# richa-batra/ParticleRobotSimulations

Hardware: AMD Instinct MI355X
Metric: particle-steps/sec at 10^6 bots; achieved HBM GB/s vs peak; 1/2/4/8-GPU ensemble (higher is better)
Workload: dtype f32

## Files before the change

### include/particlebot_hip.h

```cpp
#ifndef PARTICLEBOT_HIP_H
#define PARTICLEBOT_HIP_H

#include <stddef.h>

#include "particlebot_kernel.h"

#ifdef __cplusplus
extern "C" {
#endif

struct pbGraphicsResource;

enum { PB_RNG_COUNTER = 0, PB_RNG_XORWOW_CURAND = 1, PB_RNG_XORWOW_ROCRAND = 2 };

typedef struct pbRngState {
  unsigned d;
  unsigned v[5];
  int boxmuller_flag;
  int kind;
  float boxmuller_extra;
  float reserved[3];
} pbRngState;

int pbSetRngKind(int kind);
// ... 36 lines not shown
void updateCol(float *rad, float *col, int nCells, float *pos, float *phase, int *dead);
void collide(float *newVel, float *absForce_a, float *absForce_r, float *sortedPos, float *sortedVel,
             float *sortedRad, uint *gridParticlebotIndex, uint *cellStart, uint *cellEnd, uint nCells,
             uint numCells, float deltaTime);
void calcCOG(float *pos, float *temppos, float *temppos1, int nCells, float time, int hist_steps,
             float hist_int);
void sortParticlebots(uint *dGridParticlebotHash, uint *dGridParticlebotIndex, uint nCells);


typedef struct pbSim pbSim;

enum {
  PB_OK = 0,
  PB_ERR_HIP = 1,
  PB_ERR_ARG = 2,
  PB_ERR_NO_DEVICE = 3
};

typedef struct pbSimStats {
  unsigned long long steps;
  unsigned long long fused_launches;
  unsigned long long plain_launches;
  unsigned long long state_launches;
  unsigned long long resorts;
  unsigned long long phase_updates;
  unsigned long long resident_launches;
} pbSimStats;

const char *pbGetLastErrorString(void);

int pbGetDevice(int *device);
int pbSetDevice(int device);
int pbDevicePciBusId(int device, char *out, int cap);

int pbSimCreate(pbSim **out, const SimParams *params, float wallHalf);
void pbSimDestroy(pbSim *sim);

int pbSimCreateBatch(pbSim **out, const SimParams *params, int nsims, float wallHalf);
int pbSimBatchSize(pbSim *sim, unsigned *nsims, unsigned *nbots);
int pbSimSetStateOf(pbSim *sim, unsigned member, const float *pos, const float *vel, const float *rad,
                    const float *phase, const int *dead);
int pbSimSetStateRangeOf(pbSim *sim, unsigned member, unsigned start, unsigned count, const float *pos,
                         const float *vel, const float *rad, const float *phase, const int *dead);
int pbSimGetStateOf(pbSim *sim, unsigned member, float *pos, float *vel, float *rad, float *phase, int *dead,
                    float *absForce_a, float *absForce_r);
int pbSimGetLayoutOf(pbSim *sim, unsigned member, unsigned *orig, unsigned *keys, int *sorted);
int pbSimSetLayoutOf(pbSim *sim, unsigned member, const unsigned *orig, const unsigned *keys);
int pbSimSetForcesOf(pbSim *sim, unsigned member, const float *absForce_a, const float *absForce_r);
int pbSimCentroids(pbSim *sim, double *cxcy);
int pbSimCentroidSums(pbSim *sim, float *sumxy);
int pbSimGetColorsOf(pbSim *sim, unsigned member, float *rgba);
int pbSimSetCentroidTrail(pbSim *sim, int on);
int pbSimGetCentroidTrailOf(pbSim *sim, unsigned member, float *xy, float *times, unsigned *records);

int pbSimSetState(pbSim *sim, const float *pos, const float *vel, const float *rad, const float *phase,
                  const int *dead);
int pbSimGetState(pbSim *sim, float *pos, float *vel, float *rad, float *phase, int *dead,
                  float *absForce_a, float *absForce_r);
int pbSimSetTime(pbSim *sim, float time);
int pbSimGetTime(pbSim *sim, float *time);
int pbSimGetPhaseDraws(pbSim *sim, unsigned *draws);
int pbSimSetPhaseDraws(pbSim *sim, unsigned draws);

int pbSimStep(pbSim *sim, float deltaTime, float sort_interval, int nsteps, int *steps_done);
int pbSimStepTimed(pbSim *sim, float deltaTime, float sort_interval, int nsteps, int *steps_done,
                   float *elapsed_ms);
int pbSimStepTimedWall(pbSim *sim, float deltaTime, float sort_interval, int nsteps, int *steps_done,
                       float *elapsed_ms, double *wall_ms);
int pbSimSynchronize(pbSim *sim);

int pbSimCentroid(pbSim *sim, double *cx, double *cy);
int pbSimGetStats(pbSim *sim, pbSimStats *stats);
int pbSimSetResortEveryStep(pbSim *sim, int on);

int pbSimSetMinDistanceMode(pbSim *sim, int mode);
int pbSetMinDistanceMode(int mode);
int pbGetMinDistanceMode(void);

float pbHostSqrtThreshold(float c);

int pbSimSetForceVariant(pbSim *sim, int variant);
int pbSimSetForceSums(pbSim *sim, int mode);
int pbSimSetLanesPerBot(pbSim *sim, int lanes);
int pbSimSetResident(pbSim *sim, int mode);

int pbSimSetRng(pbSim *sim, int kind);
int pbSimGetRngStatesOf(pbSim *sim, unsigned member, pbRngState *states);

typedef struct pbForceForm {
  int flat;
  int lanes_per_bot;
  int attraction_sums;
  int offsets64;
} pbForceForm;
int pbForceFormCount(void);
int pbForceFormGet(int index, pbForceForm *form);
int pbSimSelectForceForm(pbSim *sim, int index);
int pbSimForceKernelName(pbSim *sim, char *buf, size_t cap);
int pbForceFormKernelName(int index, int payload, char *buf, size_t cap);

int pbSimSetStreamWalk(pbSim *sim, int mode);
int pbSimGetStreamWalkTrips(pbSim *sim, unsigned long long *row_by_row, unsigned long long *flattened);

typedef struct pbSimConfig {
  int force_variant;
  int force_kind;
  int lanes_per_bot;
  int resident;
  int fast_math_ok;
  int payload;
  int rng;
  int offsets64;
  int attraction_sums;
  int dead_sum_form;
  int stream_walk;
} pbSimConfig;
int pbSimGetConfig(pbSim *sim, pbSimConfig *cfg);

typedef struct pbClockSample pbClockSample;
int pbClockSampleBegin(pbClockSample **out, double seconds);
int pbClockSampleEnd(pbClockSample *sample, double *mhz, double *seconds_sampled);

int pbSelfTest(unsigned long long div_samples, unsigned long long *sqrt_checked,
               unsigned long long *sqrt_mismatches, unsigned long long *div_checked,
               unsigned long long *div_mismatches);

int pbSelfTestHoldThreshold(float c, unsigned long long *checked, unsigned long long *mismatches);
int pbSelfTestPairGeometry(unsigned first_slice, unsigned slices, unsigned long long *checked,
                           unsigned long long *mismatches);
int pbSelfTestDivision(unsigned first_slice, unsigned slices, unsigned long long *checked,
                       unsigned long long *mismatches);

#ifdef __cplusplus
}
#endif
#endif
```

### particlerobotsimulations_amd/__init__.py

```python
import ctypes as C

import numpy as np

from . import _capi
from ._capi import SimParams, make_params, pbSimConfig, pbSimStats

__all__ = ["Sim", "Ensemble", "DeviceArray", "legacy", "SimParams", "make_params", "library_paths", "self_test"]


def self_test(div_samples=1 << 32):
    vals = [C.c_ulonglong() for _ in range(4)]
    _capi.check(_capi.lib().pbSelfTest(int(div_samples), *[C.byref(v) for v in vals]), "pbSelfTest")
    keys = ("sqrt_checked", "sqrt_mismatches", "div_checked", "div_mismatches")
    return {k: int(v.value) for k, v in zip(keys, vals)}


def self_test_hold_threshold(c):
    checked, bad = C.c_ulonglong(), C.c_ulonglong()
    _capi.check(_capi.lib().pbSelfTestHoldThreshold(float(c), C.byref(checked), C.byref(bad)), "pbSelfTestHoldThreshold")
    return {"checked": checked.value, "mismatches": bad.value}


def self_test_pair_geometry(first_slice=0, slices=64):
    checked, bad = C.c_ulonglong(), C.c_ulonglong()
# ... 197 lines not shown
        return out

    @property
    def time(self):
        t = C.c_float()
        _capi.check(_capi.lib().pbSimGetTime(self._h, C.byref(t)))
        return t.value

    @time.setter
    def time(self, t):
        _capi.check(_capi.lib().pbSimSetTime(self._h, float(t)))

    @property
    def phase_draws(self):
        d = C.c_uint()
        _capi.check(_capi.lib().pbSimGetPhaseDraws(self._h, C.byref(d)))
        return d.value

    @phase_draws.setter
    def phase_draws(self, d):
        _capi.check(_capi.lib().pbSimSetPhaseDraws(self._h, int(d)))

    def step(self, nsteps, dt=0.01, sort_interval=180.0):
        done = C.c_int()
        _capi.check(_capi.lib().pbSimStep(self._h, dt, sort_interval, int(nsteps), C.byref(done)), "pbSimStep")
        return done.value

    def step_timed(self, nsteps, dt=0.01, sort_interval=180.0):
        done = C.c_int()
        ms = C.c_float()
        _capi.check(_capi.lib().pbSimStepTimed(self._h, dt, sort_interval, int(nsteps), C.byref(done),
                                               C.byref(ms)), "pbSimStepTimed")
        return done.value, ms.value

    def step_timed_wall(self, nsteps, dt=0.01, sort_interval=180.0):
        done, ms, wall = C.c_int(), C.c_float(), C.c_double()
        _capi.check(_capi.lib().pbSimStepTimedWall(self._h, dt, sort_interval, int(nsteps), C.byref(done), C.byref(ms),
                                                   C.byref(wall)), "pbSimStepTimedWall")
        return done.value, ms.value, wall.value

    def synchronize(self):
        _capi.check(_capi.lib().pbSimSynchronize(self._h))

    def centroid(self):
        cx, cy = C.c_double(), C.c_double()
        _capi.check(_capi.lib().pbSimCentroid(self._h, C.byref(cx), C.byref(cy)), "pbSimCentroid")
        return cx.value, cy.value

    def stats(self):
        s = pbSimStats()
        _capi.check(_capi.lib().pbSimGetStats(self._h, C.byref(s)))
        return {k: int(getattr(s, k)) for k, _ in pbSimStats._fields_}

    def config(self):
        c = pbSimConfig()
        _capi.check(_capi.lib().pbSimGetConfig(self._h, C.byref(c)))
        return {k: int(getattr(c, k)) for k, _ in pbSimConfig._fields_}

    def force_kernel_name(self):
        buf = C.create_string_buffer(2048)
        _capi.check(_capi.lib().pbSimForceKernelName(self._h, buf, len(buf)), "pbSimForceKernelName")
        return buf.value.decode()

    def set_force_variant(self, variant):
        _capi.check(_capi.lib().pbSimSetForceVariant(self._h, int(variant)))

    def set_stream_walk(self, mode):
        _capi.check(_capi.lib().pbSimSetStreamWalk(self._h, int(mode)), "pbSimSetStreamWalk")

    def stream_walk_trips(self):
        a, b = C.c_ulonglong(0), C.c_ulonglong(0)
        _capi.check(_capi.lib().pbSimGetStreamWalkTrips(self._h, C.byref(a), C.byref(b)), "pbSimGetStreamWalkTrips")
        return a.value, b.value

    def set_force_sums(self, mode):
        _capi.check(_capi.lib().pbSimSetForceSums(self._h, int(mode)))

    def select_force_form(self, index):
        _capi.check(_capi.lib().pbSimSelectForceForm(self._h, int(index)), "pbSimSelectForceForm")

    def set_lanes_per_bot(self, lanes):
        _capi.check(_capi.lib().pbSimSetLanesPerBot(self._h, int(lanes)))

    def set_resident(self, mode):
        _capi.check(_capi.lib().pbSimSetResident(self._h, int(mode)))

    def set_resort_every_step(self, on):
        _capi.check(_capi.lib().pbSimSetResortEveryStep(self._h, 1 if on else 0))

    def colors(self, member=0):
        out = np.empty((self.n, 4), np.float32)
        _capi.check(_capi.lib().pbSimGetColorsOf(self._h, int(member), _capi.np_ptr(out)), "pbSimGetColorsOf")
        return out

    def set_centroid_trail(self, on):
        _capi.check(_capi.lib().pbSimSetCentroidTrail(self._h, 1 if on else 0), "pbSimSetCentroidTrail")

    def centroid_trail(self, member=0):
        steps = int(self.params.centroid_steps)
        xy = np.empty((steps, 2), np.float32)
        times = np.empty(steps, np.float32)
        rec = C.c_uint(0)
        _capi.check(_capi.lib().pbSimGetCentroidTrailOf(self._h, int(member), _capi.np_ptr(xy), _capi.np_ptr(times),
                                                        C.byref(rec)), "pbSimGetCentroidTrailOf")
        return xy, times, int(rec.value)


class Ensemble(Sim):

    def __init__(self, params_list, wall_half=0.0, keepalive=None):
        self._keep = keepalive
        self.nsims = len(params_list)
        arr = (SimParams * self.nsims)(*params_list)
        self.params = params_list[0]
        self.n = int(params_list[0].nCells)
        h = C.c_void_p()
        _capi.check(_capi.lib().pbSimCreateBatch(C.byref(h), arr, self.nsims, float(wall_half)), "pbSimCreateBatch")
        self._h = h

    def set_state_of(self, member, pos=None, vel=None, rad=None, phase=None, dead=None):
        n = self.n
        pos = self._in(pos, np.float32, 2 * n)
        vel = self._in(vel, np.float32, 2 * n)
        rad = self._in(rad, np.float32, n)
        phase = self._in(phase, np.float32, n)
        dead = self._in(dead, np.int32, n)
        _capi.check(_capi.lib().pbSimSetStateOf(self._h, int(member), _capi.np_ptr(pos), _capi.np_ptr(vel),
                                                _capi.np_ptr(rad), _capi.np_ptr(phase), _capi.np_ptr(dead)),
                    "pbSimSetStateOf")

    def get_state_of(self, member):
        n = self.n
        out = {
            "pos": np.empty((n, 2), np.float32), "vel": np.empty((n, 2), np.float32),
            "rad": np.empty(n, np.float32), "phase": np.empty(n, np.float32),
            "dead": np.empty(n, np.int32), "absForce_a": np.empty(n, np.float32),
            "absForce_r": np.empty(n, np.float32),
        }
        _capi.check(_capi.lib().pbSimGetStateOf(self._h, int(member), *[_capi.np_ptr(out[k]) for k in
                                                                        ("pos", "vel", "rad", "phase", "dead",
                                                                         "absForce_a", "absForce_r")]),
                    "pbSimGetStateOf")
        if not self.config()["attraction_sums"]:
            out["absForce_a"] = None
        return out

    def centroids(self):
        out = np.empty((self.nsims, 2), np.float64)
        _capi.check(_capi.lib().pbSimCentroids(self._h, out.ctypes.data_as(C.POINTER(C.c_double))), "pbSimCentroids")
        return out

    def centroid_sums(self):
        out = np.empty((self.nsims, 2), np.float32)
        _capi.check(_capi.lib().pbSimCentroidSums(self._h, out.ctypes.data_as(C.POINTER(C.c_float))), "pbSimCentroidSums")
        return out
```

### particlerobotsimulations_amd/_capi.py

```python
import ctypes as C
import os

import numpy as np

_PKG = os.path.dirname(os.path.abspath(__file__))
LIB_DIR = os.path.join(_PKG, "lib")
HIP_SO = os.path.join(LIB_DIR, "libparticlebot_hip.so")
HOST_SO = os.path.join(LIB_DIR, "libparticlebot_host.so")

PB_MAX_OBSTACLES = 10
PB_OK = 0


class uint2(C.Structure):
    _fields_ = [("x", C.c_uint), ("y", C.c_uint)]


class float2(C.Structure):
    _fields_ = [("x", C.c_float), ("y", C.c_float)]


class SimParams(C.Structure):
    _fields_ = [
        ("gridSize", uint2), ("numCells", C.c_uint),
        ("_pad0", C.c_uint),
        ("worldOrigin", float2), ("cellSize", float2),
        ("nCells", C.c_uint), ("nDead", C.c_int), ("maxParticlebotsPerCell", C.c_uint),
        ("gravity", C.c_float), ("spring", C.c_float), ("damping", C.c_float), ("shear", C.c_float),
        ("attraction", C.c_float), ("boundaryDamping", C.c_float), ("friction", C.c_float),
        ("massFactor", C.c_float), ("frictionFactor", C.c_float), ("radFactor", C.c_float),
        ("attractionFactor", C.c_float),
        ("constraint", C.c_float), ("constraint_contraction", C.c_float),
        ("centroid_steps", C.c_int), ("centroid_int", C.c_float), ("centroid_radius", C.c_float),
        ("light_x", C.c_float), ("light_y", C.c_float), ("phase_update_interval", C.c_float),
        ("control", C.c_int), ("config", C.c_int),
        ("min_radius", C.c_float), ("max_radius", C.c_float), ("rise_period", C.c_float),
        ("freq", C.c_float),
        ("nobstacles", C.c_int),
        ("x1obs", C.POINTER(C.c_float)), ("x2obs", C.POINTER(C.c_float)),
        ("y1obs", C.POINTER(C.c_float)), ("y2obs", C.POINTER(C.c_float)),
        ("n_cir_obstacles", C.c_int),
        ("x_cir_obs", C.POINTER(C.c_float)), ("y_cir_obs", C.POINTER(C.c_float)),
        ("r_cir_obs", C.POINTER(C.c_float)),
        ("Nx", C.c_int), ("phase_std", C.c_float), ("seed", C.c_uint),
        ("light_shadow", C.c_uint), ("testing", C.c_uint), ("constrained_contraction", C.c_uint),
        ("display_shadow", C.c_uint), ("time_to_dead", C.c_float), ("max_time", C.c_float),
    ]


class pbRngState(C.Structure):
    _fields_ = [("d", C.c_uint), ("v", C.c_uint * 5), ("boxmuller_flag", C.c_int), ("kind", C.c_int),
                ("boxmuller_extra", C.c_float), ("reserved", C.c_float * 3)]


PB_RNG_COUNTER, PB_RNG_XORWOW_CURAND, PB_RNG_XORWOW_ROCRAND = 0, 1, 2


class pbSimStats(C.Structure):
    _fields_ = [("steps", C.c_ulonglong), ("fused_launches", C.c_ulonglong),
                ("plain_launches", C.c_ulonglong), ("state_launches", C.c_ulonglong),
                ("resorts", C.c_ulonglong), ("phase_updates", C.c_ulonglong),
                ("resident_launches", C.c_ulonglong)]


class pbSimConfig(C.Structure):
    _fields_ = [("force_variant", C.c_int), ("force_kind", C.c_int), ("lanes_per_bot", C.c_int),
                ("resident", C.c_int), ("fast_math_ok", C.c_int), ("payload", C.c_int), ("rng", C.c_int), ("offsets64", C.c_int),
                ("attraction_sums", C.c_int), ("dead_sum_form", C.c_int), ("stream_walk", C.c_int)]


class pbForceForm(C.Structure):
    _fields_ = [("flat", C.c_int), ("lanes_per_bot", C.c_int), ("attraction_sums", C.c_int), ("offsets64", C.c_int)]


_VP = C.c_void_p
_F = C.c_float
_U = C.c_uint
_I = C.c_int
SYMBOLS = {
    "cudaInit": (None, [_I, _VP]),
    "cudaGLInit": (None, [_I, _VP]),
    "allocateArray": (None, [C.POINTER(_VP), C.c_size_t]),
    "freeArray": (None, [_VP]),
    "threadSync": (None, []),
    "copyArrayFromDevice": (None, [_VP, _VP, _VP, _I]),
    "copyArrayToDevice": (None, [_VP, _VP, _I, _I]),
    "registerGLBufferObject": (None, [_U, C.POINTER(_VP)]),
    "unregisterGLBufferObject": (None, [_VP]),
    "mapGLBufferObject": (_VP, [C.POINTER(_VP)]),
    "unmapGLBufferObject": (None, [_VP]),
    "pbCreateBuffer": (_U, [C.c_size_t]),
    "pbBufferSubData": (None, [_U, C.c_size_t, C.c_size_t, _VP]),
    "pbDeleteBuffer": (None, [_U]),
    "setParameters": (None, [C.POINTER(SimParams)]),
    "pbSetWallHalfExtent": (None, [_F]),
    "integrateSystem": (None, [_VP, _VP, _VP, _F, _U, _F]),
    "calcHash": (None, [_VP, _VP, _VP, _I]),
    "reorderDataAndFindCellStart": (None, [_VP] * 10 + [_U, _U]),
    "updateRad_light_wave": (None, [_VP, _VP, _VP, _VP, _VP, _F, _F, _VP, _I]),
    "curand_setup": (None, [_VP, _I]),
    "add_normal_noise": (None, [_VP, _VP, _F, _I]),
    "updatePhase": (None, [_VP, _VP, _F, _F, _F, _I]),
    "updateCol": (None, [_VP, _VP, _I, _VP, _VP, _VP]),
    "collide": (None, [_VP] * 9 + [_U, _U, _F]),
    "calcCOG": (None, [_VP, _VP, _VP, _I, _F, _I, _F]),
    "sortParticlebots": (None, [_VP, _VP, _U]),
    "pbGetLastErrorString": (C.c_char_p, []),
    "pbGetDevice": (_I, [C.POINTER(_I)]),
    "pbDevicePciBusId": (_I, [_I, C.c_char_p, _I]),
    "pbSetDevice": (_I, [_I]),
    "pbSimCreate": (_I, [C.POINTER(_VP), C.POINTER(SimParams), _F]),
    "pbSimDestroy": (None, [_VP]),
    "pbSimCreateBatch": (_I, [C.POINTER(_VP), C.POINTER(SimParams), _I, _F]),
    "pbSimBatchSize": (_I, [_VP, C.POINTER(_U), C.POINTER(_U)]),
    "pbSimSetStateOf": (_I, [_VP, _U, _VP, _VP, _VP, _VP, _VP]),
    "pbSimSetStateRangeOf": (_I, [_VP, _U, _U, _U, _VP, _VP, _VP, _VP, _VP]),
    "pbSimGetStateOf": (_I, [_VP, _U] + [_VP] * 7),
    "pbSimCentroids": (_I, [_VP, C.POINTER(C.c_double)]),
    "pbSimCentroidSums": (_I, [_VP, C.POINTER(C.c_float)]),
    "pbSimGetColorsOf": (_I, [_VP, _U, _VP]),
    "pbSimSetCentroidTrail": (_I, [_VP, _I]),
    "pbSimGetCentroidTrailOf": (_I, [_VP, _U, _VP, _VP, C.POINTER(_U)]),
    "pbSimGetLayoutOf": (_I, [_VP, _U, _VP, _VP, C.POINTER(_I)]),
    "pbSimSetLayoutOf": (_I, [_VP, _U, _VP, _VP]),
    "pbSimSetForcesOf": (_I, [_VP, _U, _VP, _VP]),
    "pbSimSetState": (_I, [_VP, _VP, _VP, _VP, _VP, _VP]),
    "pbSimGetState": (_I, [_VP] * 8),
    "pbSimSetTime": (_I, [_VP, _F]),
    "pbSimGetTime": (_I, [_VP, C.POINTER(_F)]),
    "pbSimGetPhaseDraws": (_I, [_VP, C.POINTER(_U)]),
    "pbSimSetPhaseDraws": (_I, [_VP, _U]),
    "pbSimStep": (_I, [_VP, _F, _F, _I, C.POINTER(_I)]),
    "pbSimStepTimed": (_I, [_VP, _F, _F, _I, C.POINTER(_I), C.POINTER(_F)]),
    "pbSimStepTimedWall": (_I, [_VP, _F, _F, _I, C.POINTER(_I), C.POINTER(_F), C.POINTER(C.c_double)]),
    "pbSimSynchronize": (_I, [_VP]),
    "pbSimCentroid": (_I, [_VP, C.POINTER(C.c_double), C.POINTER(C.c_double)]),
    "pbSimGetStats": (_I, [_VP, C.POINTER(pbSimStats)]),
    "pbSimSetResortEveryStep": (_I, [_VP, _I]),
    "pbSimSetMinDistanceMode": (_I, [_VP, _I]),
    "pbSetMinDistanceMode": (_I, [_I]),
    "pbGetMinDistanceMode": (_I, []),
    "pbHostSqrtThreshold": (C.c_float, [C.c_float]),
    "pbSimSetForceVariant": (_I, [_VP, _I]),
    "pbSimSetLanesPerBot": (_I, [_VP, _I]),
    "pbSimSetResident": (_I, [_VP, _I]),
    "pbSimGetConfig": (_I, [_VP, C.POINTER(pbSimConfig)]),
    "pbSimSetForceSums": (_I, [_VP, _I]),
    "pbSimSetStreamWalk": (_I, [_VP, _I]),
    "pbSimGetStreamWalkTrips": (_I, [_VP, C.POINTER(C.c_ulonglong), C.POINTER(C.c_ulonglong)]),
    "pbForceFormCount": (_I, []),
    "pbForceFormGet": (_I, [_I, C.POINTER(pbForceForm)]),
    "pbSimSelectForceForm": (_I, [_VP, _I]),
    "pbSimForceKernelName": (_I, [_VP, C.c_char_p, C.c_size_t]),
    "pbForceFormKernelName": (_I, [_I, _I, C.c_char_p, C.c_size_t]),
    "pbSimSetRng": (_I, [_VP, _I]),
    "pbSimGetRngStatesOf": (_I, [_VP, _U, _VP]),
    "pbSetRngKind": (_I, [_I]),
    "pbGetRngKind": (_I, []),
    "pbClockSampleBegin": (_I, [C.POINTER(_VP), C.c_double]),
    "pbClockSampleEnd": (_I, [_VP, C.POINTER(C.c_double), C.POINTER(C.c_double)]),
    "pbSelfTest": (_I, [C.c_ulonglong] + [C.POINTER(C.c_ulonglong)] * 4),
    "pbSelfTestHoldThreshold": (_I, [C.c_float, C.POINTER(C.c_ulonglong), C.POINTER(C.c_ulonglong)]),
    "pbSelfTestPairGeometry": (_I, [_U, _U, C.POINTER(C.c_ulonglong), C.POINTER(C.c_ulonglong)]),
    "pbSelfTestDivision": (_I, [_U, _U, C.POINTER(C.c_ulonglong), C.POINTER(C.c_ulonglong)]),
}

_lib = None


def lib():
    global _lib
    if _lib is not None:
        return _lib
    if not os.path.exists(HIP_SO):
        raise RuntimeError(
            f"{HIP_SO} not found: build it with `python -c 'import __graft_entry__ as g; g.build()'` "
            "(hipcc --offload-arch=gfx950).  There is no CPU fallback.")
    L = C.CDLL(HIP_SO, mode=C.RTLD_GLOBAL)
    for name, (res, args) in SYMBOLS.items():
        fn = getattr(L, name)
        fn.restype = res
        fn.argtypes = args
    _lib = L
    return L


def check(rc, what="call"):
    if rc != PB_OK:
        msg = lib().pbGetLastErrorString()
        raise RuntimeError(f"{what} failed (code {rc}): {msg.decode() if msg else ''}")


def np_ptr(a):
    return a.ctypes.data_as(C.c_void_p) if a is not None else None


def make_params(d):
    P = SimParams()
    keep = []
    lists = {"x1obs", "x2obs", "y1obs", "y2obs", "x_cir_obs", "y_cir_obs", "r_cir_obs"}
    for k, v in d.items():
        if k in lists:
            continue
        if k == "gridSize":
            P.gridSize = uint2(int(v[0]), int(v[1]))
        elif k == "worldOrigin":
            P.worldOrigin = float2(float(v[0]), float(v[1]))
        elif k == "cellSize":
            P.cellSize = float2(float(v[0]), float(v[1]))
        else:
            setattr(P, k, v)
    for k in lists:
        vals = list(d.get(k, []))[:PB_MAX_OBSTACLES]
        arr = (C.c_float * max(1, len(vals)))(*[float(x) for x in vals])
        keep.append(arr)
        setattr(P, k, C.cast(arr, C.POINTER(C.c_float)))
    return P, keep
```

### particlerobotsimulations_amd/csrc/pb_engine.hip

```cpp
#include <algorithm>
#include <atomic>
#include <chrono>
#include <cstring>
#include <limits>
#include <string>
#include <vector>

#include "pb_engine.hpp"
#include "pb_xorwow.hpp"

std::string &pbLastError() {
  thread_local std::string text;
  return text;
}


namespace {


__global__ __launch_bounds__(TILE) void k_state(const PbDevParams *__restrict__ params, float4 *__restrict__ pr,
                                                float2 *__restrict__ vel, const float *__restrict__ phase,
                                                const int *__restrict__ dead, const float *__restrict__ absA,
                                                const float *__restrict__ absR, uint32_t n, float time, float dt,
                                                int doRadius) {
// ... 1095 lines not shown
  const float ci = S->centroidInt[0];
  const int cs = S->centroidSteps[0];
  for (uint32_t k = 0; k < S->nsims; k++)
    if (!(S->centroidInt[k] > 0.0f) || S->centroidSteps[k] <= 0 || S->centroidInt[k] != ci || S->centroidSteps[k] != cs) {
      pbLastError() = "pbSimSetCentroidTrail: every member needs the same centroid_int > 0 and centroid_steps > 0";
      return PB_ERR_ARG;
    }
  const size_t ring = (size_t)S->nsims * (size_t)cs;
  std::vector<float2> init(ring, make_float2(-5000.0f, 0.0f));
  PB_TRY(hipMalloc((void **)&S->trail, sizeof(float2) * ring));
  PB_TRY(hipMalloc((void **)&S->trailTmp, sizeof(float2) * 2 * (size_t)S->nsims * cdiv(S->n, 64)));
  PB_TRY(hipMemcpy(S->trail, init.data(), sizeof(float2) * ring, hipMemcpyHostToDevice));
  S->trailInt = ci;
  S->trailSteps = cs;
  S->trailTimes.assign((size_t)cs, std::numeric_limits<float>::quiet_NaN());
  S->trailRecords = 0;
  return PB_OK;
}

int pbSimGetCentroidTrailOf(pbSim *S, unsigned sim, float *xy, float *times, unsigned *records) {
  if (!S || sim >= S->nsims || !S->trail) {
    pbLastError() = "pbSimGetCentroidTrailOf: null handle, member out of range or trail off";
    return PB_ERR_ARG;
  }
  useDevice(S);
  if (xy) {
    PB_TRY(hipMemcpyAsync(xy, S->trail + (size_t)sim * S->trailSteps, sizeof(float2) * S->trailSteps,
                          hipMemcpyDeviceToHost, S->stream));
    PB_TRY(hipStreamSynchronize(S->stream));
  }
  if (times) memcpy(times, S->trailTimes.data(), sizeof(float) * S->trailSteps);
  if (records) *records = S->trailRecords;
  return PB_OK;
}

int pbSimGetStats(pbSim *S, pbSimStats *stats) {
  if (!S || !stats) return PB_ERR_ARG;
  *stats = S->stats;
  return PB_OK;
}

int pbSimSetForceVariant(pbSim *S, int variant) {
  if (!S || variant < 0 || variant > 3) return PB_ERR_ARG;
  const bool becomes3 = variant == 3 && S->variant != 3;
  S->variant = variant;
  if (becomes3 && S->streamWalk < 0 && S->haveCells) {
    useDevice(S);
    return chooseStreamWalk(S);
  }
  return PB_OK;
}

int pbSimSetStreamWalk(pbSim *S, int mode) {
  if (!S || mode < -1 || mode > 1) return PB_ERR_ARG;
  S->streamWalk = mode;
  if (mode < 0 && S->variant == 3 && S->haveCells) {
    useDevice(S);
    return chooseStreamWalk(S);
  }
  return PB_OK;
}

int pbSimGetStreamWalkTrips(pbSim *S, unsigned long long *rowByRow, unsigned long long *flattened) {
  if (!S) return PB_ERR_ARG;
  if (rowByRow) *rowByRow = S->walkTripsHost[0];
  if (flattened) *flattened = S->walkTripsHost[1];
  return PB_OK;
}

int pbSimSetForceSums(pbSim *S, int mode) {
  if (!S || mode < 0 || mode > 1) return PB_ERR_ARG;
  S->forceSums = mode;
  return PB_OK;
}

int pbSimSetLanesPerBot(pbSim *S, int lanes) {
  if (!S || !(lanes == 0 || lanes == 1 || lanes == 2 || lanes == 4 || lanes == 8 || lanes == 16 || lanes == 32 ||
              lanes == 64))
    return PB_ERR_ARG;
  S->lanesPerBot = lanes;
  return PB_OK;
}

int pbSimSetResident(pbSim *S, int mode) {
  if (!S || mode < 0 || mode > 2) {
    pbLastError() = "pbSimSetResident: mode must be 0 (automatic), 1 (never) or 2 (whenever it fits)";
    return PB_ERR_ARG;
  }
  S->resident = mode;
  return PB_OK;
}

int pbSimGetConfig(pbSim *S, pbSimConfig *cfg) {
  if (!S || !cfg) return PB_ERR_ARG;
  const PbForcePlan p = pbForcePlan(S);
  cfg->force_variant = S->variant;
  cfg->force_kind = p.kind;
  cfg->lanes_per_bot = p.form;
  cfg->resident = pbResidentWanted(S) ? 1 : 0;
  cfg->fast_math_ok = S->fastOk ? 1 : 0;
  cfg->payload = S->payload ? 1 : 0;
  cfg->rng = S->rng;
  cfg->offsets64 = (!p.stream && p.big) ? 1 : 0;
  cfg->attraction_sums = attractionSumsKept(S) ? 1 : 0;
  cfg->dead_sum_form = ((cfg->resident || p.stream) ? !attractionSumsKept(S) : !p.asum) ? 1 : 0;
  cfg->stream_walk = (p.stream && pbStreamWalk(S)) ? 1 : 0;
  return PB_OK;
}

int pbGetDevice(int *device) {
  if (!device) return PB_ERR_ARG;
  PB_TRY(hipGetDevice(device));
  return PB_OK;
}

int pbSetDevice(int device) {
  PB_TRY(hipSetDevice(device));
  return PB_OK;
}

int pbDevicePciBusId(int device, char *out, int cap) {
  if (!out || cap < 13) return PB_ERR_ARG;
  PB_TRY(hipDeviceGetPCIBusId(out, cap, device));
  return PB_OK;
}

int pbSimSetMinDistanceMode(pbSim *S, int mode) {
  if (!S || mode < 0 || mode > 1) return PB_ERR_ARG;
  S->minDistanceMode = mode;
  return PB_OK;
}

int pbSetMinDistanceMode(int mode) {
  if (mode < 0 || mode > 1) return PB_ERR_ARG;
  g_minDistanceMode.store(mode, std::memory_order_release);
  return PB_OK;
}

int pbGetMinDistanceMode(void) { return minDistanceDefault(); }

float pbHostSqrtThreshold(float c) { return pbSqrtThreshold(c); }

int pbSimSetResortEveryStep(pbSim *S, int on) {
  if (!S) return PB_ERR_ARG;
  S->resortEveryStep = on != 0;
  return PB_OK;
}

}
```

### particlerobotsimulations_amd/csrc/pb_engine.hpp

```cpp
#pragma once

#include <string>
#include <vector>

#include "particlebot_hip.h"
#include "pb_device.hpp"
#include "pb_internal.hpp"

std::string &pbLastError();

#define PB_TRY(expr)                                                                                  \
  do {                                                                                                \
    hipError_t e_ = (expr);                                                                           \
    if (e_ != hipSuccess) {                                                                           \
      pbLastError() = std::string(hipGetErrorName(e_)) + " at " + __FILE__ + ":" + std::to_string(__LINE__) + \
                      " in " #expr;                                                                   \
      return PB_ERR_HIP;                                                                              \
    }                                                                                                 \
  } while (0)

#ifndef PB_TILE
#define PB_TILE 256
#endif
constexpr int TILE = PB_TILE;

static inline uint32_t cdiv(uint32_t a, uint32_t b) { return (a + b - 1) / b; }

struct pbSim {
  std::vector<PbDevParams> hP;
  PbDevParams *dP = nullptr;
  SimParams host;
  uint32_t nsims = 1, n = 0, total = 0;
  int device = 0;
  hipStream_t stream = nullptr;
  hipEvent_t ev0 = nullptr, ev1 = nullptr;

  float4 *pr[2] = {nullptr, nullptr};
  float2 *vel[2] = {nullptr, nullptr};
  float *phase[2] = {nullptr, nullptr};
  int *dead[2] = {nullptr, nullptr};
  float *absA[2] = {nullptr, nullptr};
  float *absR[2] = {nullptr, nullptr};
  uint32_t *orig[2] = {nullptr, nullptr};
  int cur = 0;

  uint32_t *cellS = nullptr;
  uint32_t *keys[2] = {nullptr, nullptr}, *vals[2] = {nullptr, nullptr}, *hist = nullptr, *slotOf = nullptr;
  uint32_t *sortedKeys = nullptr;
  std::vector<uint32_t> layoutOrig, layoutKeys;
  std::vector<char> layoutGiven;
  pbRngState *rngState = nullptr;
  uint32_t *dMin = nullptr;
  float *dMinD = nullptr;
  uint32_t *hMin = nullptr;
  float *hMinD = nullptr;
  char *stage = nullptr;
  float2 *comPos = nullptr;
  double2 *comPartial = nullptr, *comOut = nullptr;
  double2 *hCom = nullptr;

  float time = 0.0f;
  uint32_t phaseDraws = 0;
  bool haveCells = false;
  bool resortEveryStep = false;
  bool payload = false, fastOk = false;
  bool xcdMembers = true;
  bool xcdTilesAll = true;
  bool magOk = false;
  int variant = 2;
  int resident = 0;
  int lanesPerBot = 0;
  int streamWalk = -1;
  bool streamWalkAuto = false;
  unsigned long long *walkTrips = nullptr, walkTripsHost[2] = {0, 0};
  bool wideOffsets = false;
  unsigned debugLdsBytes = 0;
  int rng = 0;
  int minDistanceMode = 0;
  std::vector<float> hostPos;
  int forceSums = 0;
  bool anyConstrained = false;
  std::vector<uint32_t> displayShadow;
  std::vector<float> centroidInt;
  std::vector<int> centroidSteps;
  float4 *colors = nullptr;
  float2 *trail = nullptr;
  float2 *trailTmp = nullptr;
  float trailInt = 0.0f;
  int trailSteps = 0;
  std::vector<float> trailTimes;
  unsigned trailRecords = 0;
  pbSimStats stats{};
};

static inline dim3 gridOf(const pbSim *S) { return dim3(cdiv(S->n, TILE), S->nsims); }

static inline void useDevice(const pbSim *S) { (void)hipSetDevice(S->device); }

static inline bool pbStreamWalk(const pbSim *S) { return S->streamWalk >= 0 ? S->streamWalk == 1 : S->streamWalkAuto; }
static inline bool attractionSumsKept(const pbSim *S) { return S->forceSums != 0 || S->anyConstrained; }

struct PbForcePlan {
  bool stream;
  int kind;
  int form;
  bool asum;
  bool big;
};
PbForcePlan pbForcePlan(const pbSim *S);

void pbLaunchForce(pbSim *S, bool fuse, int c, int o, float dt, float tNext, int doRadiusNext);
void pbLaunchForceStream(pbSim *S, bool fuse, int c, int o, float dt, float tNext, int doRadiusNext);
std::string pbKernelArgs(const char *mangledPointerType);
std::string pbForceStreamName(const pbSim *S);
bool pbResidentWanted(const pbSim *S);
void pbLaunchResident(pbSim *S, float dt, float t0, int m, int lightWave);
```

### particlerobotsimulations_amd/csrc/pb_force.hip

```cpp
#include <cxxabi.h>

#include <algorithm>
#include <cstdlib>
#include <cstring>
#include <typeinfo>

#include "pb_engine.hpp"

#ifdef PB_TIMELINE
__device__ unsigned long long *pbTimelineBuf = nullptr;
#define PB_TL_STAMP(word)                                                                              \
  do {                                                                                                 \
    if (pbTimelineBuf && threadIdx.x == 0)                                                             \
      pbTimelineBuf[8ull * (blockIdx.y * gridDim.x + blockIdx.x) + (word)] = __builtin_amdgcn_s_memrealtime(); \
  } while (0)
#endif

#include "pb_sweep.hpp"

namespace {

template <bool PAYLOAD, bool FLAT, int L, int NB, bool BIG, bool ASUM>
__global__ __launch_bounds__(TILE, (NB == 2 ? PB_NB2_WAVES : PB_FORCE_WAVES)) void k_force(const PbDevParams *__restrict__ params,
                                                const float4 *__restrict__ prIn, const float2 *__restrict__ velIn,
                                                const uint32_t *__restrict__ cellSAll, float *__restrict__ absR,
                                                uint32_t n, uint32_t perXcd, uint32_t memberTiles, uint32_t nsims,
                                                float dt, int fastOk,
                                                float4 *__restrict__ prOut, float2 *__restrict__ velOut,
                                                const float *__restrict__ phase, const int *__restrict__ dead,
                                                float *__restrict__ absA, const uint32_t *__restrict__ orig,
                                                float timeNext, int doRadiusNext, int fuse) {
  uint32_t member = blockIdx.y, tileX = blockIdx.x;
  if (memberTiles) {
    const uint32_t r = blockIdx.x >> 3;
    member = (r / memberTiles) * 8u + (blockIdx.x & 7u);
    tileX = r % memberTiles;
    if (member >= nsims) return;
  }
  const PbDevParams &P = params[member];
  const uint32_t tile = perXcd ? (tileX & 7u) * perXcd + (tileX >> 3) : tileX;
  const uint32_t l = tile * (TILE / L) + threadIdx.x / L;
  const uint32_t sub = threadIdx.x % L;
#ifdef PB_TIMELINE
  PB_TL_STAMP(0);
#endif
  if (l >= n) return;
  const uint32_t s = member * n + l;
  const uint32_t *__restrict__ cellS = cellSAll + (size_t)member * (P.numCells + 1u);

  const float4 me = prIn[s];
  float2 v = velIn[s];
  bool selfPayload = false;
  if (PAYLOAD) selfPayload = (orig[s] == P.nCells - 1u);
  const float att1 = selfPayload ? P.attractionFactor : 1.0f;

  PbForce F;
  F.fx = 0.0f;
  F.fy = 0.0f;
  F.fa = 0.0f;
  F.fr = 0.0f * absR[s];

  using OffT = typename std::conditional<BIG, uint64_t, uint32_t>::type;
  static_assert(ASUM || (FLAT && NB == 1), "the dead-sum form exists for the branch-free sweeps only");
  constexpr bool REPLIST = L == 1 && FLAT && NB == 1 && (!ASUM || PB_ASUM_XY);
  __shared__ float repLds[REPLIST ? (PB_REP_CAP + 1) * TILE : 1];
  float *const repCol = &repLds[REPLIST ? threadIdx.x : 0];
  if (FLAT && fastOk && __all(pbLaneFastMathOk(me.x, me.y)))
    pbSweep<PAYLOAD, FLAT, true, L, NB, OffT, ASUM>(P, prIn, velIn, cellS, 0u, s, sub, me, v, att1, F, repCol);
  else
    pbSweep<PAYLOAD, FLAT, false, L, NB, OffT, ASUM>(P, prIn, velIn, cellS, 0u, s, sub, me, v, att1, F, repCol);
  pbObstacles(P, me.x, me.y, v.x, v.y, me.z, F);
  pbFrictionAndKick(P, selfPayload, F.fx, F.fy, dt, v.x, v.y);

  float4 out = me;
  if (fuse) {
    if (doRadiusNext) out.z = pbActuate(P, me.z, phase[s], dead[s], F.fa, F.fr, timeNext, dt);
    pbIntegrate(P, out.x, out.y, v.x, v.y, out.z, dt);
  }
  if (sub == 0) {
    prOut[s] = out;
    velOut[s] = v;
    if (ASUM) absA[s] = F.fa;
    absR[s] = F.fr;
  }
#ifdef PB_TIMELINE
  if (pbTimelineBuf && threadIdx.x == 0) {
    unsigned long long *row = pbTimelineBuf + 8ull * (blockIdx.y * gridDim.x + blockIdx.x);
    row[1] = __builtin_amdgcn_s_memrealtime();
    row[2] = __builtin_amdgcn_s_getreg((20 << 0) | (0 << 6) | (3 << 11));
    row[3] = __builtin_amdgcn_s_getreg((4 << 0) | (0 << 6) | (31 << 11));
  }
#endif
}

template <bool PAYLOAD, bool FLAT, int L, bool BIG, bool ASUM>
void launchForceT(pbSim *S, bool fuse, int c, int o, float dt, float tNext, int doRadiusNext) {
  const uint32_t tiles = cdiv(S->n, TILE / L);
  const uint32_t perXcd = ((L == 1 || S->xcdTilesAll) && tiles >= 64u) ? cdiv(tiles, 8u) : 0u;
  dim3 grid(perXcd ? perXcd * 8u : tiles, S->nsims);
  uint32_t memberTiles = 0u;
  if (S->xcdMembers && !perXcd && S->nsims >= 8u) {
    memberTiles = tiles;
    grid = dim3(cdiv(S->nsims, 8u) * 8u * tiles, 1u);
  }
  constexpr int NB = (FLAT && L == 1 && !BIG && ASUM) ? PB_THROUGHPUT_NB : 1;
  const bool magNeeded = ASUM && FLAT && L == 1 && PB_ASUM_XY;
  const int fastOk = (S->variant >= 2 && S->fastOk && (!magNeeded || S->magOk)) ? 1 : 0;
  hipLaunchKernelGGL((k_force<PAYLOAD, FLAT, L, NB, BIG, ASUM>), grid, dim3(TILE), S->debugLdsBytes, S->stream, S->dP,
                     S->pr[c], S->vel[c], S->cellS, S->absR[c], S->n, perXcd, memberTiles, S->nsims, dt, fastOk, S->pr[o],
                     S->vel[o], S->phase[c], S->dead[c], S->absA[c], S->orig[c], tNext, doRadiusNext, (int)fuse);
}

template <bool PAYLOAD, bool FLAT, int L, bool BIG, bool ASUM>
std::string forceNameT() {
  constexpr int NB = (FLAT && L == 1 && !BIG && ASUM) ? PB_THROUGHPUT_NB : 1;
  auto b = [](bool v) { return std::string(v ? "true" : "false"); };
  return "k_force<" + b(PAYLOAD) + ", " + b(FLAT) + ", " + std::to_string(L) + ", " + std::to_string(NB) + ", " + b(BIG) +
         ", " + b(ASUM) + ">" + pbKernelArgs(typeid(&k_force<PAYLOAD, FLAT, L, NB, BIG, ASUM>).name());
}

using LaunchFn = void (*)(pbSim *, bool, int, int, float, float, int);
using NameFn = std::string (*)();
struct FormRow {
  pbForceForm form;
  LaunchFn launch[2];
  NameFn name[2];
};
#define PB_FORM(FL, LL, AS, BG)                                                        \
  {{FL, LL, AS, BG}, {launchForceT<false, (FL) != 0, LL, (BG) != 0, (AS) != 0>,        \
                      launchForceT<true, (FL) != 0, LL, (BG) != 0, (AS) != 0>},        \
                     {forceNameT<false, (FL) != 0, LL, (BG) != 0, (AS) != 0>,          \
                      forceNameT<true, (FL) != 0, LL, (BG) != 0, (AS) != 0>}}
const FormRow kForms[] = {
    PB_FORM(0, 1, 1, 0),
    PB_FORM(1, 1, 1, 0),  PB_FORM(1, 1, 0, 0),
    PB_FORM(1, 1, 1, 1),  PB_FORM(1, 1, 0, 1),
    PB_FORM(1, 2, 1, 0),  PB_FORM(1, 2, 0, 0),
    PB_FORM(1, 4, 1, 0),  PB_FORM(1, 4, 0, 0),
    PB_FORM(1, 8, 1, 0),  PB_FORM(1, 8, 0, 0),
    PB_FORM(1, 16, 1, 0), PB_FORM(1, 16, 0, 0),
    PB_FORM(1, 32, 1, 0), PB_FORM(1, 32, 0, 0),
    PB_FORM(1, 64, 1, 0), PB_FORM(1, 64, 0, 0),
};
#undef PB_FORM
constexpr int kNumForms = (int)(sizeof(kForms) / sizeof(kForms[0]));

}

PbForcePlan pbForcePlan(const pbSim *S) {
  PbForcePlan p{false, 0, 1, true, false};
  if (S->variant == 3 && S->total < (1u << 28) - 4u &&
      (S->lanesPerBot == 1 || (S->lanesPerBot == 0 && S->total > 131072u))) {
    p.stream = true;
    p.kind = 3;
    return p;
  }
  p.kind = S->variant == 0 ? 0 : (S->variant == 1 || !S->fastOk) ? 1 : 2;
  if (p.kind != 0) {
    p.big = S->total >= (1u << 28) - 8u || S->wideOffsets;
    const int want = p.big ? 1 : S->lanesPerBot;
    if (want == 64 || (want == 0 && S->total <= 1280u)) p.form = 64;
    else if (want == 32 || (want == 0 && S->total <= 2560u)) p.form = 32;
    else if (want == 16 || (want == 0 && S->total <= 8192u)) p.form = 16;
    else if (want == 8 || (want == 0 && S->total <= 40960u)) p.form = 8;
    else if (want == 4 || (want == 0 && S->total <= 131072u)) p.form = 4;
    else if (want == 2) p.form = 2;
    if (PB_THROUGHPUT_NB == 1 && !attractionSumsKept(S)) p.asum = false;
  }
  return p;
}

std::string pbKernelArgs(const char *mangledPointerType) {
  int status = 0;
  char *d = abi::__cxa_demangle(mangledPointerType, nullptr, nullptr, &status);
  std::string t = (status == 0 && d) ? d : mangledPointerType;
  free(d);
  const size_t at = t.find("(*)");
  return at == std::string::npos ? t : t.substr(at + 3);
}

void pbLaunchForce(pbSim *S, bool fuse, int c, int o, float dt, float tNext, int doRadiusNext) {
  const PbForcePlan plan = pbForcePlan(S);
  if (plan.stream) return pbLaunchForceStream(S, fuse, c, o, dt, tNext, doRadiusNext);
  for (const FormRow &r : kForms)
    if (r.form.flat == (plan.kind != 0) && r.form.lanes_per_bot == plan.form && (r.form.attraction_sums != 0) == plan.asum &&
        (r.form.offsets64 != 0) == plan.big)
      return r.launch[S->payload ? 1 : 0](S, fuse, c, o, dt, tNext, doRadiusNext);
  pbLastError() = "pbLaunchForce: no kernel form for this plan";
}

extern "C" {

int pbForceFormCount(void) { return kNumForms; }

int pbForceFormGet(int index, pbForceForm *form) {
  if (index < 0 || index >= kNumForms || !form) return PB_ERR_ARG;
  *form = kForms[index].form;
  return PB_OK;
}

int pbForceFormKernelName(int index, int payload, char *buf, size_t cap) {
  if (index < 0 || index >= kNumForms || !buf) return PB_ERR_ARG;
  const std::string name = kForms[index].name[payload ? 1 : 0]();
  if (name.size() + 1 > cap) return PB_ERR_ARG;
  memcpy(buf, name.c_str(), name.size() + 1);
  return PB_OK;
}

int pbSimForceKernelName(pbSim *S, char *buf, size_t cap) {
  if (!S || !buf || cap == 0) return PB_ERR_ARG;
  const PbForcePlan plan = pbForcePlan(S);
  std::string name;
  if (plan.stream) name = pbForceStreamName(S);
  for (const FormRow &r : kForms)
    if (!plan.stream && r.form.flat == (plan.kind != 0) && r.form.lanes_per_bot == plan.form &&
        (r.form.attraction_sums != 0) == plan.asum && (r.form.offsets64 != 0) == plan.big)
      name = r.name[S->payload ? 1 : 0]();
  if (name.empty() || name.size() + 1 > cap) return PB_ERR_ARG;
  memcpy(buf, name.c_str(), name.size() + 1);
  return PB_OK;
}

int pbSimSelectForceForm(pbSim *S, int index) {
  if (!S || index < -1 || index >= kNumForms) return PB_ERR_ARG;
  if (index < 0) {
    S->variant = 2;
    S->lanesPerBot = 0;
    S->forceSums = 0;
    S->wideOffsets = false;
    S->resident = 0;
    return PB_OK;
  }
  const pbForceForm &f = kForms[index].form;
  if (!f.attraction_sums && S->anyConstrained) {
    pbLastError() = "pbSimSelectForceForm: a member reads absForce_a (constrained_contraction); the dead-sum forms cannot run";
    return PB_ERR_ARG;
  }
  S->variant = f.flat ? 2 : 0;
  S->lanesPerBot = f.lanes_per_bot;
  S->forceSums = f.attraction_sums;
  S->wideOffsets = f.offsets64 != 0;
  S->resident = 1;
  return PB_OK;
}

#ifdef PB_TIMELINE
int pbDebugSetTimeline(unsigned long long *deviceBuffer) {
  return hipMemcpyToSymbol(HIP_SYMBOL(pbTimelineBuf), &deviceBuffer, sizeof deviceBuffer) == hipSuccess ? PB_OK : PB_ERR_HIP;
}
#endif

}
```

### particlerobotsimulations_amd/csrc/pb_sweep.hpp

```cpp
#pragma once

#include <type_traits>

#include "pb_device.hpp"
#include "pb_engine.hpp"

#ifndef PB_FORCE_WAVES
#define PB_FORCE_WAVES 1
#endif
#ifndef PB_NB2_WAVES
#define PB_NB2_WAVES 8
#endif
#ifndef PB_THROUGHPUT_NB
#define PB_THROUGHPUT_NB 1
#endif
#ifndef PB_PREFETCH_DEPTH
#define PB_PREFETCH_DEPTH 1
#endif
#ifndef PB_REP_CAP
#define PB_REP_CAP 8
#endif

#ifndef PB_ASUM_XY
#define PB_ASUM_XY 1
#endif
#ifndef PB_LAZY_VEL
#define PB_LAZY_VEL 1
#endif
#ifndef PB_SWEEP_EXPERIMENT
#define PB_SWEEP_EXPERIMENT 0
#endif
#ifndef PB_TL_STAMP
#define PB_TL_STAMP(word) do { } while (0)
#endif

template <int L>
__device__ __forceinline__ float pbShr1(float v) {
  if (L <= 16)
    return __int_as_float(__builtin_amdgcn_update_dpp(0, __float_as_int(v), 0x111 , 0xF, 0xF, false));
  return __int_as_float(__builtin_amdgcn_update_dpp(0, __float_as_int(v), 0x138 , 0xF, 0xF, false));
}
template <int L>
__device__ __forceinline__ float pbGroupLast(float v) {
  if (L == 64) return __int_as_float(__builtin_amdgcn_readlane(__float_as_int(v), 63));
  constexpr int PAT = ((L - 1) << 5) | (0x1F & ~(L - 1));
  return __int_as_float(__builtin_amdgcn_ds_swizzle(__float_as_int(v), PAT));
}
template <int L>
__device__ __forceinline__ void pbGroupSum(bool live, const PbPairTerm &t, PbForce &F) {
  const float tx = live ? t.tx : 0.0f, ty = live ? t.ty : 0.0f;
  const float ta = (live && !t.contact) ? t.mag : 0.0f, tr = (live && t.contact) ? t.mag : 0.0f;
  float ax = F.fx + tx, ay = F.fy + ty, aa = F.fa + ta, ar = F.fr + tr;
#pragma unroll
  for (int e = 1; e < L; e++) {
    ax = pbShr1<L>(ax) + tx;
    ay = pbShr1<L>(ay) + ty;
    aa = pbShr1<L>(aa) + ta;
    ar = pbShr1<L>(ar) + tr;
  }
  F.fx = pbGroupLast<L>(ax);
  F.fy = pbGroupLast<L>(ay);
  F.fa = pbGroupLast<L>(aa);
  F.fr = pbGroupLast<L>(ar);
}

template <int L>
__device__ __forceinline__ void pbGroupSum1(float t, float &f) {
  float a = f + t;
#pragma unroll
  for (int e = 1; e < L; e++) a = pbShr1<L>(a) + t;
  f = pbGroupLast<L>(a);
}
template <int L>
__device__ __forceinline__ void pbGroupSumXY(bool live, const PbPairXY &t, PbForce &F) {
  const float tx = live ? t.tx : 0.0f, ty = live ? t.ty : 0.0f;
  float ax = F.fx + tx, ay = F.fy + ty;
#pragma unroll
  for (int e = 1; e < L; e++) {
    ax = pbShr1<L>(ax) + tx;
    ay = pbShr1<L>(ay) + ty;
  }
  F.fx = pbGroupLast<L>(ax);
  F.fy = pbGroupLast<L>(ay);
}

struct PbSegList {
  uint32_t o0, o1, o2, o3, o4, o5, o6, o7, o8, o9;
  uint32_t c1, c2, c3, c4, c5, c6, c7, c8, c9;
  __device__ __forceinline__ void set(int r, uint32_t off, uint32_t start) {
    switch (r) {
      case 0: o0 = off; break;
      case 1: o1 = off, c1 = start; break;
      case 2: o2 = off, c2 = start; break;
      case 3: o3 = off, c3 = start; break;
      case 4: o4 = off, c4 = start; break;
      case 5: o5 = off, c5 = start; break;
      case 6: o6 = off, c6 = start; break;
      case 7: o7 = off, c7 = start; break;
      case 8: o8 = off, c8 = start; break;
      default: o9 = off, c9 = start; break;
    }
  }
};
__device__ __forceinline__ uint32_t pbSegSlot(const PbSegList SL, uint32_t m, uint32_t self, uint32_t k) {
  uint32_t o = SL.o0;
// ... 381 lines not shown
```

Baseline: 10.54 billion.

## Split last per-XCD force tiles into multi-lane tail workgroups to balance load

In the flat one-lane-per-bot force kernel with XCD-interleaved tiling, the last few tiles on each XCD are now split into smaller workgroups that use two lanes per bot. This shortens the wave-quantisation tail at the end of the force launch. The tail count defaults to one workgroup per CU per XCD and is only enabled when there are enough tiles. The launch-bounds occupancy hint for this kernel form also changes to a new wave count. The change adds a second templated sweep instantiation, which raises code size, and could perturb register allocation.

```diff
diff --git a/include/particlebot_hip.h b/include/particlebot_hip.h
--- a/include/particlebot_hip.h
+++ b/include/particlebot_hip.h
@@ -142,6 +142,8 @@
 int pbSimSetForceVariant(pbSim *sim, int variant);
 int pbSimSetForceSums(pbSim *sim, int mode);
 int pbSimSetLanesPerBot(pbSim *sim, int lanes);
+int pbSimSetTailTiles(pbSim *sim, int tiles);
+int pbForceXcdTile(unsigned workgroup, unsigned per_xcd, unsigned tail_tiles, unsigned *first_bot, unsigned *bots);
 int pbSimSetResident(pbSim *sim, int mode);
 
 int pbSimSetRng(pbSim *sim, int kind);
@@ -174,6 +176,8 @@
   int attraction_sums;
   int dead_sum_form;
   int stream_walk;
+  int tail_tiles;
+  int tail_lanes;
 } pbSimConfig;
 int pbSimGetConfig(pbSim *sim, pbSimConfig *cfg);
 
diff --git a/particlerobotsimulations_amd/__init__.py b/particlerobotsimulations_amd/__init__.py
--- a/particlerobotsimulations_amd/__init__.py
+++ b/particlerobotsimulations_amd/__init__.py
@@ -303,6 +303,9 @@
     def set_lanes_per_bot(self, lanes):
         _capi.check(_capi.lib().pbSimSetLanesPerBot(self._h, int(lanes)))
 
+    def set_tail_tiles(self, tiles):
+        _capi.check(_capi.lib().pbSimSetTailTiles(self._h, int(tiles)), "pbSimSetTailTiles")
+
     def set_resident(self, mode):
         _capi.check(_capi.lib().pbSimSetResident(self._h, int(mode)))
 
diff --git a/particlerobotsimulations_amd/_capi.py b/particlerobotsimulations_amd/_capi.py
--- a/particlerobotsimulations_amd/_capi.py
+++ b/particlerobotsimulations_amd/_capi.py
@@ -66,7 +66,8 @@
 class pbSimConfig(C.Structure):
     _fields_ = [("force_variant", C.c_int), ("force_kind", C.c_int), ("lanes_per_bot", C.c_int),
                 ("resident", C.c_int), ("fast_math_ok", C.c_int), ("payload", C.c_int), ("rng", C.c_int), ("offsets64", C.c_int),
-                ("attraction_sums", C.c_int), ("dead_sum_form", C.c_int), ("stream_walk", C.c_int)]
+                ("attraction_sums", C.c_int), ("dead_sum_form", C.c_int), ("stream_walk", C.c_int),
+                ("tail_tiles", C.c_int), ("tail_lanes", C.c_int)]
 
 
 class pbForceForm(C.Structure):
@@ -143,6 +144,8 @@
     "pbHostSqrtThreshold": (C.c_float, [C.c_float]),
     "pbSimSetForceVariant": (_I, [_VP, _I]),
     "pbSimSetLanesPerBot": (_I, [_VP, _I]),
+    "pbSimSetTailTiles": (_I, [_VP, _I]),
+    "pbForceXcdTile": (_I, [_U, _U, _U, C.POINTER(_U), C.POINTER(_U)]),
     "pbSimSetResident": (_I, [_VP, _I]),
     "pbSimGetConfig": (_I, [_VP, C.POINTER(pbSimConfig)]),
     "pbSimSetForceSums": (_I, [_VP, _I]),
diff --git a/particlerobotsimulations_amd/csrc/pb_engine.hip b/particlerobotsimulations_amd/csrc/pb_engine.hip
--- a/particlerobotsimulations_amd/csrc/pb_engine.hip
+++ b/particlerobotsimulations_amd/csrc/pb_engine.hip
@@ -1201,6 +1201,12 @@
   return PB_OK;
 }
 
+int pbSimSetTailTiles(pbSim *S, int tiles) {
+  if (!S || tiles < -1) return PB_ERR_ARG;
+  S->tailTiles = tiles;
+  return PB_OK;
+}
+
 int pbSimSetResident(pbSim *S, int mode) {
   if (!S || mode < 0 || mode > 2) {
     pbLastError() = "pbSimSetResident: mode must be 0 (automatic), 1 (never) or 2 (whenever it fits)";
@@ -1224,6 +1230,8 @@
   cfg->attraction_sums = attractionSumsKept(S) ? 1 : 0;
   cfg->dead_sum_form = ((cfg->resident || p.stream) ? !attractionSumsKept(S) : !p.asum) ? 1 : 0;
   cfg->stream_walk = (p.stream && pbStreamWalk(S)) ? 1 : 0;
+  cfg->tail_tiles = (int)pbForceTailTiles(S);
+  cfg->tail_lanes = cfg->tail_tiles ? PB_TAIL_LANES : 0;
   return PB_OK;
 }
 
diff --git a/particlerobotsimulations_amd/csrc/pb_engine.hpp b/particlerobotsimulations_amd/csrc/pb_engine.hpp
--- a/particlerobotsimulations_amd/csrc/pb_engine.hpp
+++ b/particlerobotsimulations_amd/csrc/pb_engine.hpp
@@ -73,6 +73,8 @@
   int streamWalk = -1;
   bool streamWalkAuto = false;
   unsigned long long *walkTrips = nullptr, walkTripsHost[2] = {0, 0};
+  uint32_t cuCount = 0;
+  int tailTiles = -1;
   bool wideOffsets = false;
   unsigned debugLdsBytes = 0;
   int rng = 0;
@@ -108,6 +110,19 @@
   bool big;
 };
 PbForcePlan pbForcePlan(const pbSim *S);
+#ifndef PB_TAIL_LANES
+#define PB_TAIL_LANES 2
+#endif
+__host__ __device__ inline bool pbXcdTile(uint32_t tileX, uint32_t perXcd, uint32_t tail, uint32_t &first) {
+  const uint32_t x = tileX & 7u, k = tileX >> 3, mainK = perXcd - tail;
+  if (k < mainK) {
+    first = (x * perXcd + k) * TILE;
+    return false;
+  }
+  first = (x * perXcd + mainK) * TILE + (k - mainK) * (TILE / PB_TAIL_LANES);
+  return true;
+}
+uint32_t pbForceTailTiles(pbSim *S);
 
 void pbLaunchForce(pbSim *S, bool fuse, int c, int o, float dt, float tNext, int doRadiusNext);
 void pbLaunchForceStream(pbSim *S, bool fuse, int c, int o, float dt, float tNext, int doRadiusNext);
diff --git a/particlerobotsimulations_amd/csrc/pb_force.hip b/particlerobotsimulations_amd/csrc/pb_force.hip
--- a/particlerobotsimulations_amd/csrc/pb_force.hip
+++ b/particlerobotsimulations_amd/csrc/pb_force.hip
@@ -21,7 +21,7 @@
 namespace {
 
 template <bool PAYLOAD, bool FLAT, int L, int NB, bool BIG, bool ASUM>
-__global__ __launch_bounds__(TILE, (NB == 2 ? PB_NB2_WAVES : PB_FORCE_WAVES)) void k_force(const PbDevParams *__restrict__ params,
+__global__ __launch_bounds__(TILE, (NB == 2 ? PB_NB2_WAVES : (L == 1 && FLAT && !BIG && !PAYLOAD) ? PB_TAIL_FORM_WAVES : PB_FORCE_WAVES)) void k_force(const PbDevParams *__restrict__ params,
                                                 const float4 *__restrict__ prIn, const float2 *__restrict__ velIn,
                                                 const uint32_t *__restrict__ cellSAll, float *__restrict__ absR,
                                                 uint32_t n, uint32_t perXcd, uint32_t memberTiles, uint32_t nsims,
@@ -31,16 +31,26 @@
                                                 float *__restrict__ absA, const uint32_t *__restrict__ orig,
                                                 float timeNext, int doRadiusNext, int fuse) {
   uint32_t member = blockIdx.y, tileX = blockIdx.x;
-  if (memberTiles) {
+  if (memberTiles && !perXcd) {
     const uint32_t r = blockIdx.x >> 3;
     member = (r / memberTiles) * 8u + (blockIdx.x & 7u);
     tileX = r % memberTiles;
     if (member >= nsims) return;
   }
   const PbDevParams &P = params[member];
-  const uint32_t tile = perXcd ? (tileX & 7u) * perXcd + (tileX >> 3) : tileX;
-  const uint32_t l = tile * (TILE / L) + threadIdx.x / L;
-  const uint32_t sub = threadIdx.x % L;
+  uint32_t tile = perXcd ? (tileX & 7u) * perXcd + (tileX >> 3) : tileX;
+  uint32_t l = tile * (TILE / L) + threadIdx.x / L;
+  uint32_t sub = threadIdx.x % L;
+  constexpr bool TAILABLE = L == 1 && FLAT && NB == 1 && !BIG;
+  bool tailWg = false;
+  if (TAILABLE && perXcd && memberTiles) {
+    uint32_t first;
+    tailWg = pbXcdTile(tileX, perXcd, memberTiles, first);
+    if (tailWg) {
+      l = first + threadIdx.x / PB_TAIL_LANES;
+      sub = threadIdx.x % PB_TAIL_LANES;
+    }
+  }
 #ifdef PB_TIMELINE
   PB_TL_STAMP(0);
 #endif
@@ -65,10 +75,17 @@
   constexpr bool REPLIST = L == 1 && FLAT && NB == 1 && (!ASUM || PB_ASUM_XY);
   __shared__ float repLds[REPLIST ? (PB_REP_CAP + 1) * TILE : 1];
   float *const repCol = &repLds[REPLIST ? threadIdx.x : 0];
-  if (FLAT && fastOk && __all(pbLaneFastMathOk(me.x, me.y)))
-    pbSweep<PAYLOAD, FLAT, true, L, NB, OffT, ASUM>(P, prIn, velIn, cellS, 0u, s, sub, me, v, att1, F, repCol);
+  auto sweep = [&](auto lanes) __attribute__((always_inline)) {
+    constexpr int LS = decltype(lanes)::value;
+    if (FLAT && fastOk && __all(pbLaneFastMathOk(me.x, me.y)))
+      pbSweep<PAYLOAD, FLAT, true, LS, NB, OffT, ASUM>(P, prIn, velIn, cellS, 0u, s, sub, me, v, att1, F, repCol);
+    else
+      pbSweep<PAYLOAD, FLAT, false, LS, NB, OffT, ASUM>(P, prIn, velIn, cellS, 0u, s, sub, me, v, att1, F, repCol);
+  };
+  if (TAILABLE && tailWg)
+    sweep(std::integral_constant<int, TAILABLE ? PB_TAIL_LANES : L>{});
   else
-    pbSweep<PAYLOAD, FLAT, false, L, NB, OffT, ASUM>(P, prIn, velIn, cellS, 0u, s, sub, me, v, att1, F, repCol);
+    sweep(std::integral_constant<int, L>{});
   pbObstacles(P, me.x, me.y, v.x, v.y, me.z, F);
   pbFrictionAndKick(P, selfPayload, F.fx, F.fy, dt, v.x, v.y);
 
@@ -93,17 +110,30 @@
 #endif
 }
 
+uint32_t pbTailTiles(pbSim *S, uint32_t perXcd) {
+  if (S->tailTiles >= 0) return std::min((uint32_t)S->tailTiles, perXcd);
+  if (S->cuCount == 0) {
+    int cus = 0;
+    if (hipDeviceGetAttribute(&cus, hipDeviceAttributeMultiprocessorCount, S->device) != hipSuccess || cus <= 0) cus = 256;
+    S->cuCount = (uint32_t)cus;
+  }
+  const uint32_t cusPerXcd = std::max(S->cuCount / 8u, 1u);
+  const uint32_t wgPerCu = PB_TAIL_FORM_WAVES * 4u / (TILE / 64u);
+  return perXcd >= cusPerXcd * wgPerCu ? cusPerXcd : 0u;
+}
+
 template <bool PAYLOAD, bool FLAT, int L, bool BIG, bool ASUM>
 void launchForceT(pbSim *S, bool fuse, int c, int o, float dt, float tNext, int doRadiusNext) {
   const uint32_t tiles = cdiv(S->n, TILE / L);
   const uint32_t perXcd = ((L == 1 || S->xcdTilesAll) && tiles >= 64u) ? cdiv(tiles, 8u) : 0u;
-  dim3 grid(perXcd ? perXcd * 8u : tiles, S->nsims);
-  uint32_t memberTiles = 0u;
+  constexpr int NB = (FLAT && L == 1 && !BIG && ASUM) ? PB_THROUGHPUT_NB : 1;
+  const uint32_t tail = (FLAT && L == 1 && NB == 1 && !BIG && perXcd) ? pbTailTiles(S, perXcd) : 0u;
+  dim3 grid(perXcd ? (perXcd + tail * (PB_TAIL_LANES - 1)) * 8u : tiles, S->nsims);
+  uint32_t memberTiles = tail;
   if (S->xcdMembers && !perXcd && S->nsims >= 8u) {
     memberTiles = tiles;
     grid = dim3(cdiv(S->nsims, 8u) * 8u * tiles, 1u);
   }
-  constexpr int NB = (FLAT && L == 1 && !BIG && ASUM) ? PB_THROUGHPUT_NB : 1;
   const bool magNeeded = ASUM && FLAT && L == 1 && PB_ASUM_XY;
   const int fastOk = (S->variant >= 2 && S->fastOk && (!magNeeded || S->magOk)) ? 1 : 0;
   hipLaunchKernelGGL((k_force<PAYLOAD, FLAT, L, NB, BIG, ASUM>), grid, dim3(TILE), S->debugLdsBytes, S->stream, S->dP,
@@ -147,6 +177,13 @@
 
 }
 
+uint32_t pbForceTailTiles(pbSim *S) {
+  const PbForcePlan p = pbForcePlan(S);
+  if (p.stream || p.kind == 0 || p.form != 1 || p.big || pbResidentWanted(S)) return 0u;
+  const uint32_t tiles = cdiv(S->n, TILE);
+  return tiles >= 64u ? pbTailTiles(S, cdiv(tiles, 8u)) : 0u;
+}
+
 PbForcePlan pbForcePlan(const pbSim *S) {
   PbForcePlan p{false, 0, 1, true, false};
   if (S->variant == 3 && S->total < (1u << 28) - 4u &&
@@ -191,6 +228,15 @@
 
 extern "C" {
 
+int pbForceXcdTile(unsigned workgroup, unsigned per_xcd, unsigned tail_tiles, unsigned *first_bot, unsigned *bots) {
+  if (!first_bot || !bots || tail_tiles > per_xcd || workgroup >= 8u * (per_xcd + tail_tiles * (PB_TAIL_LANES - 1u)))
+    return PB_ERR_ARG;
+  uint32_t first;
+  *bots = pbXcdTile(workgroup, per_xcd, tail_tiles, first) ? TILE / PB_TAIL_LANES : TILE;
+  *first_bot = first;
+  return PB_OK;
+}
+
 int pbForceFormCount(void) { return kNumForms; }
 
 int pbForceFormGet(int index, pbForceForm *form) {
diff --git a/particlerobotsimulations_amd/csrc/pb_sweep.hpp b/particlerobotsimulations_amd/csrc/pb_sweep.hpp
--- a/particlerobotsimulations_amd/csrc/pb_sweep.hpp
+++ b/particlerobotsimulations_amd/csrc/pb_sweep.hpp
@@ -21,6 +21,9 @@
 #define PB_REP_CAP 8
 #endif
 
+#ifndef PB_TAIL_FORM_WAVES
+#define PB_TAIL_FORM_WAVES 8
+#endif
 #ifndef PB_ASUM_XY
 #define PB_ASUM_XY 1
 #endif
```

Result: faster. 11.00 billion, median of 6 (+4.4%).
